# vnminin/phylomap

Measured on NVIDIA B200. Metric: sampled branch-site histories/sec (4-state, 10k-tip tree), higher is better.
Workload: dtype f32

## Files before the change

phylomap_b200/csrc/pm_device.cuh:

```cuda
#pragma once
#include <cstdint>
#include <cuda_runtime.h>

#define PM_NMAX 32
#define PM_DIC_NMAX 8
#define PM_LOCAL_PATH_MAX 64
#define PM_SMEM_POW 8

#define PM_DE_SAMPLE_NA 1u
#define PM_DE_SAMPLE_NEG 2u
#define PM_DE_SAMPLE_ZERO 4u
#define PM_DE_PATH_CAP 8u
#define PM_DE_M_OVERFLOW 16u
#define PM_DE_REPLAY 32u
#define PM_DE_INCONSISTENT 64u
#define PM_DE_BAD_STATE 128u
#define PM_DE_JUMP_LIMIT 256u

namespace pm {

template <typename Real, bool EXACT> struct Ar;
template <> struct Ar<double, true> {
  static __device__ __forceinline__ double mul(double a, double b) { return __dmul_rn(a, b); }
  static __device__ __forceinline__ double add(double a, double b) { return __dadd_rn(a, b); }
// ... 107 lines not shown
    return ((float)(x >> 8) + 0.5f) * (1.0f / 16777216.0f);
  }
};

template <typename Real, bool EXACT> struct StreamSel { typedef StreamD type; };
template <> struct StreamSel<float, false> { typedef StreamF type; };

__device__ __forceinline__ double exp_rand_R(StreamD& g) {
  const double q[16] = {0.6931471805599453, 0.9333736875190459, 0.9888777961838675, 0.9984589039328340,
                        0.9998292811061389, 0.9999833164100727, 0.9999985691438767, 0.9999998906925558,
                        0.9999999924734159, 0.9999999995283275, 0.9999999999728814, 0.9999999999985598,
                        0.9999999999999289, 0.9999999999999968, 0.9999999999999999, 1.0000000000000000};
  double a = 0.;
  double u = g.next();
  while (u <= 0. || u >= 1.) u = g.next();
  for (;;) {
    u = __dadd_rn(u, u);
    if (u > 1.) break;
    a = __dadd_rn(a, q[0]);
  }
  u = __dsub_rn(u, 1.);
  if (u <= q[0]) return __dadd_rn(a, u);
  int i = 0;
  double ustar = g.next(), umin = ustar;
  do {
    ustar = g.next();
    if (umin > ustar) umin = ustar;
    i++;
  } while (u > q[i]);
  return __dadd_rn(a, __dmul_rn(umin, q[0]));
}

template <typename Real, bool EXACT> struct ExpDev;
template <> struct ExpDev<double, true> {
  static __device__ __forceinline__ double draw(StreamD& g) { return exp_rand_R(g); }
};
template <> struct ExpDev<double, false> {
  static __device__ __forceinline__ double draw(StreamD& g) { return -log(g.next()); }
};
template <> struct ExpDev<float, false> {
  static __device__ __forceinline__ float draw(StreamF& g) { return -logf(g.next()); }
};

#define PM_LAMBDA_INV 16

template <typename Real> struct Pin;
template <> struct Pin<float> {
  static __device__ __forceinline__ float mul(float a, float b) { return __fmul_rn(a, b); }
  static __device__ __forceinline__ float add(float a, float b) { return __fadd_rn(a, b); }
  static __device__ __forceinline__ float sub(float a, float b) { return __fsub_rn(a, b); }
  static __device__ __forceinline__ float div(float a, float b) { return __fdiv_rn(a, b); }
  static __device__ __forceinline__ float u01(uint32_t w) { return __fmaf_rn((float)(w >> 9), 1.0f / 8388608.0f, 1.0f / 16777216.0f); }
  static __device__ __forceinline__ float expm(float x) {
    float r;
    asm("ex2.approx.ftz.f32 %0, %1;" : "=f"(r) : "f"(__fmul_rn(x, -1.4426950216293334961f)));
    return r;
  }
  static __device__ __forceinline__ float root(float u, int k) {
    float l, r;
    asm("lg2.approx.ftz.f32 %0, %1;" : "=f"(l) : "f"(u));
    asm("ex2.approx.ftz.f32 %0, %1;" : "=f"(r) : "f"(__fdiv_rn(l, (float)k)));
    return r;
  }
  static __device__ __forceinline__ float neglog(float u) { return -logf(u); }
  static __device__ __forceinline__ int above3(float u, float a, float b, float c) {
    unsigned x, y, z;
    asm("set.gt.u32.f32 %0, %1, %2;" : "=r"(x) : "f"(u), "f"(a));
    asm("set.gt.u32.f32 %0, %1, %2;" : "=r"(y) : "f"(u), "f"(b));
    asm("set.gt.u32.f32 %0, %1, %2;" : "=r"(z) : "f"(u), "f"(c));
    return -(int)(x + y + z);
  }
};
template <> struct Pin<double> {
  static __device__ __forceinline__ double mul(double a, double b) { return __dmul_rn(a, b); }
  static __device__ __forceinline__ double add(double a, double b) { return __dadd_rn(a, b); }
  static __device__ __forceinline__ double sub(double a, double b) { return __dsub_rn(a, b); }
  static __device__ __forceinline__ double div(double a, double b) { return __ddiv_rn(a, b); }
  static __device__ __forceinline__ double u01(uint32_t w) { return ((double)w + 0.5) * (1.0 / 4294967296.0); }
  static __device__ __forceinline__ double expm(double x) { return exp(-x); }
  static __device__ __forceinline__ double root(double u, int k) { return exp2(__ddiv_rn(log2(u), (double)k)); }
  static __device__ __forceinline__ double neglog(double u) { return -log(u); }
  static __device__ __forceinline__ int above3(double u, double a, double b, double c) { return (u > a ? 1 : 0) + (u > b ? 1 : 0) + (u > c ? 1 : 0); }
};

__constant__ float pm_recip[65] = {
    0.f, 1.f, 1.f / 2, 1.f / 3, 1.f / 4, 1.f / 5, 1.f / 6, 1.f / 7, 1.f / 8, 1.f / 9, 1.f / 10, 1.f / 11, 1.f / 12, 1.f / 13,
    1.f / 14, 1.f / 15, 1.f / 16, 1.f / 17, 1.f / 18, 1.f / 19, 1.f / 20, 1.f / 21, 1.f / 22, 1.f / 23, 1.f / 24, 1.f / 25,
    1.f / 26, 1.f / 27, 1.f / 28, 1.f / 29, 1.f / 30, 1.f / 31, 1.f / 32, 1.f / 33, 1.f / 34, 1.f / 35, 1.f / 36, 1.f / 37,
    1.f / 38, 1.f / 39, 1.f / 40, 1.f / 41, 1.f / 42, 1.f / 43, 1.f / 44, 1.f / 45, 1.f / 46, 1.f / 47, 1.f / 48, 1.f / 49,
    1.f / 50, 1.f / 51, 1.f / 52, 1.f / 53, 1.f / 54, 1.f / 55, 1.f / 56, 1.f / 57, 1.f / 58, 1.f / 59, 1.f / 60, 1.f / 61,
    1.f / 62, 1.f / 63, 1.f / 64};

template <typename Real>
__device__ __forceinline__ int poisson_inv(Real lam, uint32_t word) {
  typedef Pin<Real> PN;
  const Real u = PN::u01(word);
  const Real p0 = PN::expm(lam);
  const Real p1 = PN::mul(p0, lam);
  const Real p2 = PN::mul(PN::mul(p1, lam), (Real)0.5);
  const Real c1 = PN::add(p0, p1), c2 = PN::add(c1, p2);
  int k = Pin<Real>::above3(u, p0, c1, c2);
  if (k == 3) {
    Real p = p2, c = c2;
    k = 2;
    while (u > c && k < 64) {
      k++;
      p = PN::mul(PN::mul(p, lam), (Real)pm_recip[k]);
      c = PN::add(c, p);
      if (p < (Real)1e-12 && (Real)k > lam) break;
    }
  }
  return k;
}

template <typename Real>
__device__ __forceinline__ Real next_order_stat(Real x, Real L, int remaining, uint32_t word) {
  const Real u = Pin<Real>::u01(word);
  const Real frac = Pin<Real>::sub((Real)1, remaining == 1 ? u : Pin<Real>::root(u, remaining));
  return Pin<Real>::add(x, Pin<Real>::mul(Pin<Real>::sub(L, x), frac));
}

template <typename Real>
__device__ __forceinline__ Real pos_dec(uint32_t q, Real Le) { return Pin<Real>::mul((Real)q, Pin<Real>::mul(Le, (Real)(1.0 / 65536.0))); }
template <typename Real>
__device__ __forceinline__ uint32_t pos_enc(Real p, Real Le) {
  const Real f = Pin<Real>::add(Pin<Real>::mul(p, Pin<Real>::div((Real)65536, Le)), (Real)0.5);
  return (uint32_t)min(max((int)f, 0), 65535);
}
__device__ __forceinline__ uint32_t pos_rand(uint32_t word) { return min(((word >> 15) + 1u) >> 1, 65535u); }
#define PM_SHAPE(nj, s0, s1) ((uint16_t)((uint32_t)(nj) | ((uint32_t)(s0) << 6) | ((uint32_t)(s1) << 11)))

struct WordStream {
  uint32_t k0, k1, site, iter, slot, hi, j;
  uint32_t o0, o1, o2, o3;
  __device__ __forceinline__ void open(const RngDesc& d, uint32_t local_site, uint32_t it, uint32_t kind, uint32_t idx, uint32_t run) {
    k0 = d.k0; k1 = d.k1; site = d.site0 + local_site; iter = it; slot = make_slot(kind, idx); hi = run << 20; j = 0;
  }
  __device__ __forceinline__ uint32_t next() {
    const uint32_t q = j & 3u;
    if (q == 0u) {
      uint32_t o[4];
      philox4x32_10(hi | (j >> 2), slot, iter, site, k0, k1, o);
      o0 = o[0]; o1 = o[1]; o2 = o[2]; o3 = o[3];
    }
    j++;
    return q == 0u ? o0 : q == 1u ? o1 : q == 2u ? o2 : o3;
  }
};

__device__ __forceinline__ void pair_block(const RngDesc& d, uint32_t local_site, uint32_t it, uint32_t e, uint32_t o[4]) {
  philox4x32_10_rk(e >> 1, make_slot(K_BRPAIR, 0u), it, d.site0 + local_site, d.rk, o);
}

template <typename Real, int NC, bool EXACT, typename U>
__device__ __forceinline__ int categorical(const Real* w, int n, U u, unsigned* err) {
  if (EXACT) {
    Real sum = 0; int npos = 0; unsigned bad = 0;
#pragma unroll
    for (int i = 0; i < n; i++) {
      Real v = w[i];
      if (!isfinite(v)) bad |= PM_DE_SAMPLE_NA;
      else if (v < (Real)0) bad |= PM_DE_SAMPLE_NEG;
      if (v > (Real)0) { npos++; sum = Ar<Real, true>::add(sum, v); }
    }
    if (npos == 0) bad |= PM_DE_SAMPLE_ZERO;
    if (bad) { atomicOr(err, bad); return 0; }
    Real p[NC]; int perm[NC];
#pragma unroll
    for (int i = 0; i < n; i++) { p[i] = Ar<Real, true>::div(w[i], sum); perm[i] = i; }
#pragma unroll
    for (int i = 1; i < n; i++) {
#pragma unroll
      for (int j = i; j >= 1; j--) {
        if (p[j] > p[j - 1]) {
          Real tp = p[j]; p[j] = p[j - 1]; p[j - 1] = tp;
          int ti = perm[j]; perm[j] = perm[j - 1]; perm[j - 1] = ti;
        }
      }
    }
    Real c = 0;
    int pick = -1;
    const int last = perm[n - 1];
#pragma unroll
    for (int j = 0; j < n - 1; j++) {
      c = (j == 0) ? p[0] : Ar<Real, true>::add(c, p[j]);
      if (pick < 0 && (double)u <= (double)c) pick = perm[j];
    }
    return pick < 0 ? last : pick;
  } else {
    Real tot = 0;
#pragma unroll
    for (int i = 0; i < n; i++) tot += w[i];
    if (!(tot > (Real)0) || !isfinite(tot)) { atomicOr(err, tot > (Real)0 ? PM_DE_SAMPLE_NA : PM_DE_SAMPLE_ZERO); return 0; }
    Real t = (Real)u * tot, c = 0;
    int pick = -1, lastpos = 0;
#pragma unroll
    for (int i = 0; i < n; i++) {
      c += w[i];
      if (w[i] > (Real)0) lastpos = i;
      if (pick < 0 && t < c && w[i] > (Real)0) pick = i;
    }
    return pick < 0 ? lastpos : pick;
  }
}

template <typename Real, int NC, bool EXACT>
__device__ __forceinline__ void matvec(const Real* __restrict__ M, int n, Real* v) {
  Real y[NC];
#pragma unroll
  for (int i = 0; i < n; i++) {
    Real acc = 0;
#pragma unroll
    for (int j = 0; j < n; j++) acc = Ar<Real, EXACT>::add(acc, Ar<Real, EXACT>::mul(M[i * n + j], v[j]));
    y[i] = acc;
  }
#pragma unroll
  for (int i = 0; i < n; i++) v[i] = y[i];
}
template <typename Real, int NC, bool EXACT>
__device__ __forceinline__ void matvec_t(const Real* __restrict__ M, int n, Real* v) {
  Real y[NC];
#pragma unroll
  for (int j = 0; j < n; j++) {
    Real acc = 0;
#pragma unroll
    for (int i = 0; i < n; i++) acc = Ar<Real, EXACT>::add(acc, Ar<Real, EXACT>::mul(M[i * n + j], v[i]));
    y[j] = acc;
  }
#pragma unroll
  for (int j = 0; j < n; j++) v[j] = y[j];
}

template <typename Real, int NS> struct VecIO {
  static __device__ __forceinline__ void load(const Real* p, int n, Real* v) { for (int i = 0; i < n; i++) v[i] = p[i]; }
  static __device__ __forceinline__ void store(Real* p, int n, const Real* v) { for (int i = 0; i < n; i++) p[i] = v[i]; }
};
template <> struct VecIO<float, 4> {
  static __device__ __forceinline__ void load(const float* p, int, float* v) {
    float4 t = *reinterpret_cast<const float4*>(p); v[0] = t.x; v[1] = t.y; v[2] = t.z; v[3] = t.w; }
  static __device__ __forceinline__ void store(float* p, int, const float* v) {
    *reinterpret_cast<float4*>(p) = make_float4(v[0], v[1], v[2], v[3]); }
};
template <> struct VecIO<float, 2> {
  static __device__ __forceinline__ void load(const float* p, int, float* v) {
    float2 t = *reinterpret_cast<const float2*>(p); v[0] = t.x; v[1] = t.y; }
  static __device__ __forceinline__ void store(float* p, int, const float* v) {
    *reinterpret_cast<float2*>(p) = make_float2(v[0], v[1]); }
};
template <> struct VecIO<double, 4> {
  static __device__ __forceinline__ void load(const double* p, int, double* v) {
    double2 a = reinterpret_cast<const double2*>(p)[0], b = reinterpret_cast<const double2*>(p)[1];
    v[0] = a.x; v[1] = a.y; v[2] = b.x; v[3] = b.y; }
  static __device__ __forceinline__ void store(double* p, int, const double* v) {
    reinterpret_cast<double2*>(p)[0] = make_double2(v[0], v[1]); reinterpret_cast<double2*>(p)[1] = make_double2(v[2], v[3]); }
};
template <> struct VecIO<double, 2> {
  static __device__ __forceinline__ void load(const double* p, int, double* v) {
    double2 a = *reinterpret_cast<const double2*>(p); v[0] = a.x; v[1] = a.y; }
  static __device__ __forceinline__ void store(double* p, int, const double* v) {
    *reinterpret_cast<double2*>(p) = make_double2(v[0], v[1]); }
};

}
```

phylomap_b200/csrc/pm_kernels.cuh:

```cuda
#pragma once
#include <type_traits>
#include "pm_device.cuh"

namespace pm {

template <typename Real>
struct ChainParams {
  int n, T, E;
  const int* cap_off;
  long long S;
  const Real* model;
  const Real* ppow;
  int jcap;
  const int* up_entries; const int* up_off; int n_up_levels;
  int* rec_cursor;
  const int* cl_entries; const int* cl_warp_off; const int* cl_top_entries; const int* cl_top_off; int n_cl_top_levels;
  const int* cd_top; const int* cd_top_off; int n_cd_top_levels; const int* cd_entries; const int* cd_warp_off;
  const long long* cd_tips; int n_cd_tips;
  const int* down_entries; const int* down_off; int n_down_levels;
  const int* e_parent; const int* e_child; const Real* e_len;
  const long long* maps_off; const double* maps_len;
  int root;
  const uint8_t* tipcode; long long TS;
  uint8_t* node_state; uint32_t* meta; Real* PL;
// ... 774 lines not shown
      cp_async4(slot + PLB + lane4, reinterpret_cast<const char*>(mtb_u) + off64(q0.z, q0.w));
      if (lane < 8) cp_async4(slot + hdst, reinterpret_cast<const char*>(e) + hsrc, lane < 4 || more);
    };
#pragma unroll 1
    for (int u = 0; u < DEPTH; u++) {
      if (i0 + u < i1) { issue(ring + u * SLOT, ep, __ldg(ep), i0 + u + DEPTH < i1); ep += 4; }
      cp_async_commit();
    }
    long long vA = 0, vB = 0, pA = -1, pB = -1;
    int psA = 0, psB = 0;
    if (i0 < i1) {
      cp_async_wait<DEPTH - 1>();
      __syncwarp();
      const int4 h = lds_v4(ring + PLB + 128);
      vA = off64(h.x, h.y); pA = off64(h.z, h.w);
      if (pA >= 0) psA = *reinterpret_cast<const uint8_t*>(nsb_u + (unsigned long long)pA);
    }
    unsigned slot = ring;
    unsigned ring_end = ring + DEPTH * SLOT;
    asm volatile("" : "+r"(ring_end));
    int sprev = 0;
    uint32_t o[4] = {0, 0, 0, 0};
    auto step = [&](int idx, long long v_off, long long p_off, int ps_mem, long long& v_off_n, long long& p_off_n, int& ps_mem_n) {
      const unsigned slot_n = (slot + SLOT == ring_end) ? ring : slot + SLOT;
      cp_async_wait<DEPTH - 2>();
      __syncwarp();
      if (idx + 1 < i1) {
        const int4 h = lds_v4(slot_n + PLB + 128);
        v_off_n = off64(h.x, h.y); p_off_n = off64(h.z, h.w);
        if (h.w >= 0) ps_mem_n = *reinterpret_cast<const uint8_t*>(nsb_u + (unsigned long long)p_off_n);
      }
      if ((idx & 3) == 0 || idx == i0) philox4x32_10_rk((uint32_t)idx >> 2, kslot, iter, gsite, P.rng.rk, o);
      const uint32_t word = (idx & 3) == 0 ? o[0] : (idx & 3) == 1 ? o[1] : (idx & 3) == 2 ? o[2] : o[3];
      Real pl[NS];
      lds_vec<Real, NS>(slot + lanePB, pl);
      const int k = lds_u16(slot + PLB + lane4) - 1;
      const int ps = p_off < 0 ? sprev : ps_mem;
      const int sn = draw_node_state<Real, NS>(P, sBs, sPow, npow_s, k, ps, pl, word);
      if (act) *reinterpret_cast<uint8_t*>(nsb_u + (unsigned long long)v_off) = (uint8_t)sn;
      sprev = sn;
      __syncwarp();
      if (idx + DEPTH < i1) {
        const int4 q0 = lds_v4(slot + PLB + 144);
        __syncwarp();
        issue(slot, ep, q0, idx + 2 * DEPTH < i1);
        ep += 4;
      }
      cp_async_commit();
      slot = slot_n;
    };
#pragma unroll 1
    for (int idx = i0; idx < i1; idx += 2) {
      step(idx, vA, pA, psA, vB, pB, psB);
      if (idx + 1 < i1) step(idx + 1, vB, pB, psB, vA, pA, psA);
    }
    cp_async_wait<0>();
  }
  if (P.n_cd_tips > 0) {
    __syncthreads();
    const int ntip = P.n_cd_tips, ngrp = (ntip + 3) >> 2;
    const uint8_t* const tipb = P.tipcode + site;
    const char* const mtb = reinterpret_cast<const char*>(P.meta + site);
    struct TipLoad { int ps, k, cd; };
    auto load = [&](int grp, TipLoad (&L)[4]) {
#pragma unroll
      for (int q = 0; q < 4; q++) {
        const int v = min(4 * grp + q, ntip - 1);
        const longlong2 en = __ldg(reinterpret_cast<const longlong2*>(P.cd_tips) + v);
        L[q].ps = nst[en.x];
        L[q].k = (int)(*reinterpret_cast<const uint32_t*>(mtb + en.y) & 0xffffu) - 1;
        L[q].cd = tipb[(long long)v * P.TS];
      }
    };
    auto draw = [&](int grp, const TipLoad (&L)[4]) {
      uint32_t o[4];
      philox4x32_10_rk(0x40000000u + (uint32_t)grp, kslot, iter, gsite, P.rng.rk, o);
#pragma unroll
      for (int q = 0; q < 4; q++) {
        if (4 * grp + q < ntip) {
          const uint32_t word = q == 0 ? o[0] : q == 1 ? o[1] : q == 2 ? o[2] : o[3];
          const int sn = draw_tip_state<Real, NS>(P, sBs, sPow, npow_s, L[q].k, L[q].ps, L[q].cd, parity, word);
          if (active) nst[(long long)(4 * grp + q) * S] = (uint8_t)sn;
        }
      }
    };
    TipLoad A[4], B[4];
    int grp = warp;
    if (grp < ngrp) load(grp, A);
    while (grp < ngrp) {
      if (grp + nw < ngrp) load(grp + nw, B);
      draw(grp, A);
      grp += nw;
      if (grp >= ngrp) break;
      if (grp + nw < ngrp) load(grp + nw, A);
      draw(grp, B);
      grp += nw;
    }
  }
}

template <typename Real, int NS, int DEPTH, int MINB>
__global__ void __launch_bounds__(256, MINB) k_nodes_clade(ChainParams<Real> P, uint32_t iter) {
  if (P.ctl) iter = P.ctl[0];
  nodes_clade_block<Real, NS, DEPTH>(P, iter, P.tile_base + (long long)blockIdx.x * 32, (long long)blockIdx.x * 32);
}

__device__ __forceinline__ unsigned long long global_ns() { unsigned long long t; asm volatile("mov.u64 %0, %%globaltimer;" : "=l"(t)); return t; }
__device__ __forceinline__ unsigned sm_id() { unsigned v; asm volatile("mov.u32 %0, %%smid;" : "=r"(v)); return v; }

template <typename Real, int NS, int DEPTH, int MINB>
__global__ void __launch_bounds__(256, MINB) k_prune_nodes_clade(ChainParams<Real> P, uint32_t iter, long long b0, int phases, int* slot_busy,
                                                                 int slots_per_sm, unsigned long long* phase_ns) {
  if (P.ctl) iter = P.ctl[0];
  __shared__ unsigned long long s_t[2];
  __shared__ int s_slot;
  if (threadIdx.x == 0) {
    int slot = (int)blockIdx.x;
    if (slot_busy) {
      const int base = (int)sm_id() * slots_per_sm;
      int k = 0;
      while (atomicCAS(slot_busy + base + k, 0, 1) != 0) k = (k + 1 == slots_per_sm) ? 0 : k + 1;
      slot = base + k;
    }
    s_slot = slot;
    if (phase_ns) s_t[0] = global_ns();
  }
  __syncthreads();
  const int slot = s_slot;
  const long long site0 = (b0 + blockIdx.x) * 32, pl0 = (long long)slot * 32;
  prune_clade_block<Real, NS, DEPTH>(P, site0, pl0);
  __syncthreads();
  if (phases & 2) {
    if (phase_ns && threadIdx.x == 0) s_t[1] = global_ns();
    nodes_clade_block<Real, NS, DEPTH>(P, iter, site0, pl0);
    __syncthreads();
    if (phase_ns && threadIdx.x == 0) {
      const unsigned long long t2 = global_ns();
      atomicAdd(phase_ns, s_t[1] - s_t[0]);
      atomicAdd(phase_ns + 1, t2 - s_t[1]);
    }
  }
  if (threadIdx.x == 0 && slot_busy) atomicExch(slot_busy + slot, 0);
}

#define PM_META(m, q) ((uint32_t)(m) | ((uint32_t)(q) << 16))

template <typename Real>
__device__ __forceinline__ bool rate_ok(Real r) { return isfinite(r) && r > (Real)0; }

__device__ __forceinline__ float lds_real(unsigned a, float) { float v; asm volatile("ld.shared.f32 %0, [%1];" : "=f"(v) : "r"(a)); return v; }
__device__ __forceinline__ double lds_real(unsigned a, double) { double v; asm volatile("ld.shared.f64 %0, [%1];" : "=d"(v) : "r"(a)); return v; }
__device__ __forceinline__ unsigned smem_addr(const void* p) { return (unsigned)__cvta_generic_to_shared(p); }

template <typename Real>
struct EasySmem {
  int cnt, rate, unit, topo;
  __host__ __device__ static int up16(int x) { return (x + 15) & ~15; }
  __host__ __device__ explicit EasySmem(int n) {
    cnt = up16(4 * n * (int)sizeof(double));
    rate = up16(cnt + n * n * (int)sizeof(unsigned));
    unit = up16(rate + n * (int)sizeof(Real));
    topo = up16(unit + n * n * (int)sizeof(Real));
  }
  __host__ __device__ size_t bytes(int chunk) const { return (size_t)topo + (size_t)chunk * 16; }
};
__device__ __forceinline__ void lds_v2s32(unsigned a, int& x, int& y) { asm volatile("ld.shared.v2.s32 {%0,%1}, [%2];" : "=r"(x), "=r"(y) : "r"(a)); }
__device__ __forceinline__ void red_shared_inc(unsigned a) { asm volatile("red.shared.add.u32 [%0], 1;" ::"r"(a) : "memory"); }

template <typename Real, int NS>
__global__ void __launch_bounds__(128, (sizeof(Real) == 8 ? 6 : 8)) k_paths_easy(ChainParams<Real> P, uint32_t iter, int chunk) {
  if (P.ctl) iter = P.ctl[0];
  constexpr int NR = NS > 0 ? NS : 1;
  typedef Pin<Real> PN;
  const int n = NS > 0 ? NS : P.n;
  extern __shared__ __align__(16) unsigned char smem_raw[];
  const EasySmem<Real> lay(n);
  double* s_dw = reinterpret_cast<double*>(smem_raw);
  unsigned* s_cnt = reinterpret_cast<unsigned*>(smem_raw + lay.cnt);
  Real* s_rate = reinterpret_cast<Real*>(smem_raw + lay.rate);
  Real* s_unit = reinterpret_cast<Real*>(smem_raw + lay.unit);
  unsigned char* s_topo = smem_raw + lay.topo;
  const int e0 = blockIdx.y * chunk, e1 = min(P.E, e0 + chunk);
  for (int i = threadIdx.x; i < n * n; i += blockDim.x) { s_cnt[i] = 0; s_unit[i] = (i / n == i % n) ? (Real)1 : (Real)0; }
  for (int i = threadIdx.x; i < n; i += blockDim.x) {
    const Real r = P.model[2 * n * n + 4 * n + i];
    s_rate[i] = rate_ok(r) ? r : (Real)0;
  }
  for (int i = threadIdx.x; i < 4 * n; i += blockDim.x) s_dw[i] = 0.0;
  for (int i = threadIdx.x; i < e1 - e0; i += blockDim.x) {
    int* en = reinterpret_cast<int*>(s_topo + 16 * (size_t)i);
    en[0] = P.e_parent[e0 + i]; en[1] = P.e_child[e0 + i];
    *reinterpret_cast<Real*>(en + 2) = P.e_len[e0 + i];
  }
  __syncthreads();
  unsigned a_base = smem_addr(smem_raw);
  asm volatile("" : "+r"(a_base));
  const unsigned a_cnt = a_base + (unsigned)lay.cnt, a_rate = a_base + (unsigned)lay.rate, a_unit = a_base + (unsigned)lay.unit,
                 a_topo = a_base + (unsigned)lay.topo;
  const long long S = P.S;
  const uint32_t Su = (uint32_t)S;
  const long long site_raw = (long long)blockIdx.x * blockDim.x + threadIdx.x;
  const long long site = site_raw < S ? site_raw : S - 1;
  const bool full = P.full_counts != 0;
  const long long wglob = site_raw >> 5;
  uint32_t* __restrict__ const bal_b = P.hard_ballot + (long long)e0 * P.W + wglob;
  const bool bal_writer = (threadIdx.x & 31) == 0 && wglob < (long long)P.W;
  const uint32_t Wu = (uint32_t)P.W;
  uint32_t* __restrict__ const meta_b = P.meta + (long long)e0 * S + site;
  uint16_t* __restrict__ const shape_b = P.shape + (long long)e0 * S + site;
  uint32_t row = 0, rowf = 0, rowb = 0;
  const uint8_t* __restrict__ nstate = P.node_state + site;
  Real Racc[NR]; double Rsum[NR];
#pragma unroll
  for (int j = 0; j < NR; j++) { Racc[j] = 0; Rsum[j] = 0; }
  auto add_dwell = [&](int s, Real L) {
    if (NS > 0) {
      Real u[NR];
      lds_vec<Real, NS>(a_unit + (unsigned)s * (unsigned)(NR * sizeof(Real)), u);
#pragma unroll
      for (int j = 0; j < NR; j++) Racc[j] = fma(u[j], L, Racc[j]);
    } else if (L != (Real)0) atomicAdd(&s_dw[s], (double)L);
  };
  auto flush_dwell = [&]() {
    if (NS > 0) {
#pragma unroll
      for (int j = 0; j < NR; j++) { Rsum[j] += (double)Racc[j]; Racc[j] = 0; }
    }
  };
  const int nb = e1 - e0;
  struct Ahead { uint32_t mt; int ps, cs; };
  Ahead X = {0, 0, 0}, Y = {0, 0, 0};
  auto fetch = [&](int i, Ahead& a) {
    a.mt = meta_b[rowf]; rowf += Su;
    int par, chi;
    lds_v2s32(a_topo + 16u * (unsigned)i, par, chi);
    a.ps = nstate[(uint64_t)(uint32_t)par * Su];
    a.cs = nstate[(uint64_t)(uint32_t)chi * Su];
  };
  uint32_t po[4] = {0, 0, 0, 0};
  auto body = [&](int i, auto odd_c, auto newblk_c, auto tail_c, const Ahead cur) {
    constexpr bool ODD = decltype(odd_c)::value, NEWBLK = decltype(newblk_c)::value, TAIL = decltype(tail_c)::value;
    const int e = e0 + i;
    const uint32_t mt = cur.mt; const int ps = cur.ps, cs = cur.cs;
    if (NEWBLK) pair_block(P.rng, (uint32_t)site, iter, (uint32_t)e, po);
    const uint32_t wA = ODD ? po[2] : po[0], wB = ODD ? po[3] : po[1];
    const int m = (int)(mt & 0xffffu);
    const uint32_t q = mt >> 16;
    const Real Le = lds_real(a_topo + 16u * (unsigned)i + 8u, (Real)0);
    const bool two = (m == 2) && (ps != cs);
    const Real p1 = pos_dec<Real>(q, Le);
    const Real L0 = two ? p1 : Le;
    const int s0 = two ? ps : cs;
    const Real L1 = two ? PN::sub(Le, p1) : (Real)0;
    const Real lam = PN::add(PN::mul(lds_real(a_rate + (unsigned)sizeof(Real) * (unsigned)s0, (Real)0), L0),
                             PN::mul(lds_real(a_rate + (unsigned)sizeof(Real) * (unsigned)cs, (Real)0), L1));
    const bool hard = (m > 2) || lam > (Real)PM_LAMBDA_INV;
    const bool ok = TAIL ? (!hard && site_raw < S) : !hard;
    const int k = poisson_inv<Real>(lam, wA);
    if (ok && m == 2 && (full || two)) red_shared_inc(a_cnt + 4u * (unsigned)(ps * n + cs));
    add_dwell(s0, ok ? L0 : (Real)0);
    add_dwell(cs, ok ? L1 : (Real)0);
    const uint32_t newq = (!two && k == 1) ? pos_rand(wB) : q;
    if (ok) { meta_b[row] = PM_META((two ? 2 : 1) + k, newq); shape_b[row] = PM_SHAPE(two ? 1 : 0, s0, cs); }
    row += Su;
    const unsigned bal = __ballot_sync(0xffffffffu, TAIL ? (hard && site_raw < S) : hard);
    if (bal_writer) bal_b[rowb] = bal;
    rowb += Wu;
  };
  auto run = [&](auto tail_c) {
    const std::true_type T{}; const std::false_type F{};
    int i = 0;
    if (nb > 0 && (e0 & 1)) {
      fetch(0, X);
      body(0, T, T, tail_c, X);
      i = 1;
    }
    if (i < nb) fetch(i, X);
    if (i + 1 < nb) fetch(i + 1, Y);
    while (i + 3 < nb) {
      const int stop = min(nb - 4, i + 62);
      for (; i <= stop; i += 2) {
        const Ahead cx = X, cy = Y;
        fetch(i + 2, X); fetch(i + 3, Y);
        body(i, F, T, tail_c, cx);
        body(i + 1, T, F, tail_c, cy);
      }
      flush_dwell();
    }
    for (; i + 1 < nb; i += 2) {
      const Ahead cx = X, cy = Y;
      if (i + 2 < nb) fetch(i + 2, X);
      if (i + 3 < nb) fetch(i + 3, Y);
      body(i, F, T, tail_c, cx);
      body(i + 1, T, F, tail_c, cy);
    }
    if (i < nb) body(i, F, T, tail_c, X);
    flush_dwell();
  };
  if ((long long)(blockIdx.x + 1) * blockDim.x <= S) run(std::false_type()); else run(std::true_type());
  if (NS > 0) {
    const int lane = threadIdx.x & 31, warp = threadIdx.x >> 5;
#pragma unroll
    for (int j = 0; j < NR; j++) {
      double v = Rsum[j];
#pragma unroll
      for (int o = 16; o > 0; o >>= 1) v += __shfl_down_sync(0xffffffffu, v, o);
      if (lane == 0) s_dw[warp * n + j] = v;
    }
  }
  __syncthreads();
  const long long blk = (long long)blockIdx.y * gridDim.x + blockIdx.x;
  if ((int)threadIdx.x < n) {
    double v;
    if (NS > 0) { v = 0; for (int w = 0; w < (int)(blockDim.x >> 5); w++) v += s_dw[w * n + threadIdx.x]; }
    else v = s_dw[threadIdx.x];
    P.dw_partial[blk * n + threadIdx.x] = v;
  }
  for (int i = threadIdx.x; i < n * n; i += blockDim.x) if (s_cnt[i]) atomicAdd(&P.cnt[i], (unsigned long long)s_cnt[i]);
}

template <typename Real>
__device__ __forceinline__ Real rate_or_zero(Real r) { return rate_ok(r) ? r : (Real)0; }

template <typename Real>
struct RunPieces {
  Real L, x, rate;
  int left;
  bool gaps;
  bool firstB;
  uint32_t wB;
  WordStream ws;
  bool joint, pend, run0;
  Real v, sc;
  __device__ __forceinline__ void begin(const RngDesc& d, uint32_t site, uint32_t it, uint32_t e, int run, Real len, Real r,
                                       uint32_t cnt_word, bool single_run, uint32_t wordB) {
    L = len; x = 0; rate = r; left = 0; gaps = false; firstB = single_run; wB = wordB; joint = false;
    if (!rate_ok(r)) return;
    const Real lam = Pin<Real>::mul(r, len);
    if (lam > (Real)PM_LAMBDA_INV) { gaps = true; ws.open(d, site, it, K_BRGAP, e, (uint32_t)run); }
    else { left = poisson_inv<Real>(lam, cnt_word); ws.open(d, site, it, K_BRPOS, e, (uint32_t)run); }
  }
  __device__ __forceinline__ void begin_joint(const RngDesc& d, uint32_t site, uint32_t it, uint32_t e, Real len0, int K, Real lam0,
                                             Real lamT, Real r0, uint32_t wordB) {
    typedef Pin<Real> PN;
    L = len0; x = 0; left = K; gaps = false; firstB = true; wB = wordB; joint = true; pend = false; run0 = true;
    v = 0; rate = PN::div(lam0, lamT); sc = PN::div(lamT, r0);
    ws.open(d, site, it, K_BRPOS, e, 0u);
  }
  __device__ __forceinline__ void second_run(Real len1, Real lamT, Real r1) { L = len1; x = 0; run0 = false; sc = Pin<Real>::div(lamT, r1); }
  __device__ __forceinline__ Real next(bool& last) {
    typedef Pin<Real> PN;
    if (joint) {
      if (!pend && left > 0) {
        uint32_t w;
        if (firstB) { w = wB; firstB = false; } else w = ws.next();
        v = next_order_stat<Real>(v, (Real)1, left, w);
        left--; pend = true;
      }
      if (pend && (!run0 || v < rate)) {
        const Real t2 = min(PN::mul(run0 ? v : PN::sub(v, rate), sc), L);
        const Real piece = max(PN::sub(t2, x), (Real)0);
        x = max(t2, x); pend = false; last = false;
        return piece;
      }
      last = true;
      return PN::sub(L, x);
    }
    if (gaps) {
      const Real g = PN::div(PN::neglog(PN::u01(ws.next())), rate);
      const Real t2 = PN::add(x, g);
      if (t2 < L) { x = t2; last = false; return g; }
      last = true;
      return PN::sub(L, x);
    }
    if (left > 0) {
      uint32_t w;
      if (firstB) { w = wB; firstB = false; } else w = ws.next();
      const Real t2 = next_order_stat<Real>(x, L, left, w);
      const Real piece = PN::sub(t2, x);
      x = t2; left--; last = false;
      return piece;
    }
    last = true;
    return PN::sub(L, x);
  }
};

template <typename Real>
__device__ __noinline__ int count_gaps(RngDesc d, uint32_t site, uint32_t it, uint32_t e, uint32_t run, Real L, Real rate, Real* first) {
  typedef Pin<Real> PN;
  WordStream g; g.open(d, site, it, K_BRGAP, e, run);
  Real x = 0; int k = 0;
  for (;;) {
    const Real gp = PN::div(PN::neglog(PN::u01(g.next())), rate);
    const Real t2 = PN::add(x, gp);
    if (!(t2 < L) || k > 70000) break;
    x = t2; k++;
    if (k == 1) *first = gp;
  }
  return k;
}

template <typename Real>
struct HardItem { uint32_t site, e, meta, ends, shape; };

template <typename Real, int NS>
struct PathWorker {
  static constexpr int NC = NS > 0 ? NS : PM_NMAX;
  static constexpr int NR = NS > 0 ? NS : 1;
  typedef typename StreamSel<Real, false>::type Stream;
  typedef Pin<Real> PN;
  const ChainParams<Real>& P;
  const uint32_t iter; const int first; const int n; const bool full;
  const Real* const sB; const Real* const sBs; const Real* const sPow; const int npow_s;
  unsigned* const s_cnt; double* const s_dw;
  const Real* const s_rate_old; const Real* const s_rate_new;
  const Real* __restrict__ rd_len; const uint8_t* __restrict__ rd_st;
  Real* __restrict__ wr_len; uint8_t* __restrict__ wr_st;
  double Rsum[NR];
  unsigned errbits;
  __device__ __forceinline__ PathWorker(const ChainParams<Real>& P_, uint32_t iter_, int first_, int n_, const Real* sB_, const Real* sBs_,
                                        const Real* sPow_, int npow_s_, unsigned* s_cnt_, double* s_dw_, const Real* rate_old_,
                                        const Real* rate_new_)
      : P(P_), iter(iter_), first(first_), n(n_), full(P_.full_counts != 0), sB(sB_), sBs(sBs_), sPow(sPow_), npow_s(npow_s_),
        s_cnt(s_cnt_), s_dw(s_dw_), s_rate_old(rate_old_), s_rate_new(rate_new_), rd_len(P_.rec_len[(iter_ & 1u) ^ 1u]),
        rd_st(P_.rec_st[(iter_ & 1u) ^ 1u]), wr_len(P_.rec_len[iter_ & 1u]), wr_st(P_.rec_st[iter_ & 1u]), errbits(0) {
#pragma unroll
    for (int j = 0; j < NR; j++) Rsum[j] = 0;
  }
  __device__ __forceinline__ void add_dwell(int s, Real L) {
    if (NS > 0) {
#pragma unroll
      for (int j = 0; j < NR; j++) Rsum[j] += (s == j) ? (double)L : 0.0;
    } else atomicAdd(&s_dw[s], (double)L);
  }

  __device__ __forceinline__ void short_item(const HardItem<Real> it, uint32_t& meta_out, uint16_t& shape_out) {
    const long long site = it.site;
    const int eb = (int)it.e;
    const uint32_t mt = it.meta;
    const int m = (int)(mt & 0xffffu);
    const int nj = (int)(it.shape & 0x3fu);
    const int so0 = (int)((it.shape >> 6) & 0x1fu), so1 = (int)((it.shape >> 11) & 0x1fu);
    const int ps = (int)(it.ends & 0xffu), cs = (int)(it.ends >> 8);
    const Real Le = __ldg(P.e_len + eb);
    const uint32_t gsite = P.rng.site0 + (uint32_t)site;
    uint32_t po_old[4], po_new[4];
    pair_block(P.rng, (uint32_t)site, iter, (uint32_t)eb, po_new);
    if (nj < 2) pair_block(P.rng, (uint32_t)site, iter - 1u, (uint32_t)eb, po_old);
    const uint32_t nA = (eb & 1) ? po_new[2] : po_new[0], nB = (eb & 1) ? po_new[3] : po_new[1];
    Real J0, J1, J2;
    if (nj >= 2) {
      const int ck = eb / P.chunk;
      const int cap0 = __ldg(P.cap_off + ck), cap_c = __ldg(P.cap_off + ck + 1) - cap0;
      const long long sl = ((long long)cap0 * P.rec_groups) + (site >> P.rec_shift) * (long long)cap_c;
      const int rd0 = (int)(mt >> 16);
      J0 = rd_len[sl + min(rd0, cap_c - 1)];
// ... 442 lines not shown
```

phylomap_b200/csrc/pm_launch_impl.cuh:

```cuda
#pragma once
#include "pm_launch.cuh"

namespace pm {

template <typename Real, int NS, bool EXACT>
void Sweep<Real, NS, EXACT>::prune(const ChainParams<Real>& P, int grid, size_t smem, cudaStream_t st) {
  if constexpr (!EXACT && (NS == 2 || NS == 4)) {
    constexpr int D = 8, MB = sizeof(Real) == 8 ? 2 : 3;
    const size_t spow = 2 * PM_SMEM_POW * NS * NS * sizeof(Real);
    const size_t sm = spow + (size_t)PM_CLADE_SLOT * 8 * D;
    auto kern = k_prune_clade<Real, NS, D, MB>;
    cudaFuncSetAttribute(kern, cudaFuncAttributeMaxDynamicSharedMemorySize, (int)sm);
    kern<<<grid, 256, sm, st>>>(P);
  }
  else k_prune<Real, NS, EXACT><<<grid, 256, smem, st>>>(P);
}
template <typename Real, int NS, bool EXACT>
void Sweep<Real, NS, EXACT>::nodes(const ChainParams<Real>& P, int grid, size_t smem, cudaStream_t st, uint32_t iter) {
  if constexpr (!EXACT && (NS == 2 || NS == 4)) {
    constexpr int D = 8, MB = sizeof(Real) == 8 ? 2 : 3;
    const size_t sm = smem + (size_t)(32 * NS * sizeof(Real) + 160) * 8 * D;
    auto kern = k_nodes_clade<Real, NS, D, MB>;
    cudaFuncSetAttribute(kern, cudaFuncAttributeMaxDynamicSharedMemorySize, (int)sm);
    kern<<<grid, 256, sm, st>>>(P, iter);
  }
  else k_nodes<Real, NS, EXACT><<<grid, 256, smem, st>>>(P, iter);
}
template <typename Real, int NS, bool EXACT>
struct FusedCfg {
  static constexpr int D = 8, MB = sizeof(Real) == 8 ? 2 : 3;
  static size_t smem(size_t smem_nodes) {
    const size_t sm_prune = 2 * PM_SMEM_POW * (NS > 0 ? NS : 1) * (NS > 0 ? NS : 1) * sizeof(Real) + (size_t)PM_CLADE_SLOT * 8 * D;
    const size_t sm_nodes = smem_nodes + (size_t)(32 * (NS > 0 ? NS : 1) * sizeof(Real) + 160) * 8 * D;
    return sm_prune > sm_nodes ? sm_prune : sm_nodes;
  }
};
template <typename Real, int NS, bool EXACT>
int Sweep<Real, NS, EXACT>::fused_blocks_per_sm(size_t smem_nodes) {
  if constexpr (!EXACT && (NS == 2 || NS == 4)) {
    typedef FusedCfg<Real, NS, EXACT> C;
    auto kern = k_prune_nodes_clade<Real, NS, C::D, C::MB>;
    const size_t sm = C::smem(smem_nodes);
    cudaFuncSetAttribute(kern, cudaFuncAttributeMaxDynamicSharedMemorySize, (int)sm);
    int nb = 0;
    if (cudaOccupancyMaxActiveBlocksPerMultiprocessor(&nb, kern, 256, sm) != cudaSuccess) return 0;
    return nb;
  }
  return 0;
}
template <typename Real, int NS, bool EXACT>
void Sweep<Real, NS, EXACT>::prune_nodes(const ChainParams<Real>& P, int grid, size_t smem_nodes, cudaStream_t st, uint32_t iter,
                                         long long b0, int phases, int* slot_busy, int slots_per_sm, unsigned long long* phase_ns) {
  if constexpr (!EXACT && (NS == 2 || NS == 4)) {
    typedef FusedCfg<Real, NS, EXACT> C;
    auto kern = k_prune_nodes_clade<Real, NS, C::D, C::MB>;
    const size_t sm = C::smem(smem_nodes);
    cudaFuncSetAttribute(kern, cudaFuncAttributeMaxDynamicSharedMemorySize, (int)sm);
    kern<<<grid, 256, sm, st>>>(P, iter, b0, phases, slot_busy, slots_per_sm, phase_ns);
  }
}
template <typename Real, int NS, bool EXACT>
void Sweep<Real, NS, EXACT>::paths(const ChainParams<Real>& P, dim3 grid, size_t smem, cudaStream_t st, uint32_t iter,
                                   int first, int chunk, int hard_blocks) {
  if constexpr (EXACT) k_paths<Real, NS, true><<<grid, 128, smem, st>>>(P, iter, first, chunk);
  else {
    const size_t smem_easy = EasySmem<Real>(P.n).bytes(chunk);
    k_paths_easy<Real, NS><<<grid, 128, smem_easy, st>>>(P, iter, chunk);
    if (!first) k_paths_hard<Real, NS, 8, 0><<<2 * hard_blocks, 128, smem, st>>>(P, iter, first);
    k_paths_hard<Real, NS, 4, 1><<<hard_blocks, 128, smem, st>>>(P, iter, first);
  }
}
template <typename Real, int NS, bool EXACT>
size_t Sweep<Real, NS, EXACT>::small_smem(int T) {
  if constexpr (!EXACT && (NS == 2 || NS == 4)) return (size_t)SmallSmem<Real, NS>(T).total;
  return (size_t)1 << 40;
}
template <typename Real, int NS, bool EXACT>
void Sweep<Real, NS, EXACT>::small_chain(const ChainParams<Real>& P, int sites, cudaStream_t st, uint32_t iter0, int nsweeps,
                                         const SmallOut& out, bool two_per_sm) {
  if constexpr (!EXACT && (NS == 2 || NS == 4)) {
    const size_t sm = (size_t)SmallSmem<Real, NS>(P.T).total;
    auto kern = two_per_sm ? k_small_chain<Real, NS, 2> : k_small_chain<Real, NS, 1>;
    cudaFuncSetAttribute(kern, cudaFuncAttributeMaxDynamicSharedMemorySize, (int)sm);
    kern<<<sites, 256, sm, st>>>(P, iter0, nsweeps, out);
  }
}

}
```

Before: 68.59 billion.

## Cut register pressure in easy path kernel via smem dwell accumulators and hoisted Philox keys

Moves the per-thread dwell accumulators (Racc/Rsum) out of registers into per-thread shared-memory slots, updated with predicated load-add-store. It also replaces the one-hot unit-vector lookup and precomputes the iteration-dependent Philox rounds once per thread (PairBlocks), so each new pair block needs fewer multiplies. Topology is split into an int2 array plus a separate length array, and branches become predicated PTX loads and stores. The aim is lower register use and less divergence and RNG cost, at the price of more shared-memory traffic and a larger smem footprint per block.

```diff
diff --git a/phylomap_b200/csrc/pm_device.cuh b/phylomap_b200/csrc/pm_device.cuh
--- a/phylomap_b200/csrc/pm_device.cuh
+++ b/phylomap_b200/csrc/pm_device.cuh
@@ -283,6 +283,36 @@
   philox4x32_10_rk(e >> 1, make_slot(K_BRPAIR, 0u), it, d.site0 + local_site, d.rk, o);
 }
 
+struct PairBlocks {
+  uint32_t a, k2, k3, k5;
+  static __device__ __forceinline__ void mulw(uint32_t m, uint32_t c, uint32_t& hi, uint32_t& lo) {
+    const uint64_t p = (uint64_t)m * c;
+    hi = (uint32_t)(p >> 32); lo = (uint32_t)p;
+  }
+  __device__ __forceinline__ PairBlocks(const RngDesc& d, uint32_t it) {
+    a = __umulhi(0xCD9E8D57u, it) ^ make_slot(K_BRPAIR, 0u) ^ d.rk[0];
+    k2 = (0xCD9E8D57u * it) ^ d.rk[2];
+    k3 = __umulhi(0xD2511F53u, a) ^ d.rk[3];
+    k5 = (0xD2511F53u * a) ^ d.rk[5];
+  }
+  __device__ __forceinline__ void block(const RngDesc& d, uint32_t j, uint32_t gsite, uint32_t o[4]) const {
+    uint32_t h0, l0, h1, l1;
+    mulw(0xD2511F53u, j, h0, l0);
+    mulw(0xCD9E8D57u, h0 ^ gsite ^ d.rk[1], h1, l1);
+    uint32_t c0 = h1 ^ k2, c1 = l1, c2 = l0 ^ k3, c3;
+    mulw(0xD2511F53u, c0, h0, l0);
+    mulw(0xCD9E8D57u, c2, h1, l1);
+    c0 = h1 ^ c1 ^ d.rk[4]; c2 = h0 ^ k5; c1 = l1; c3 = l0;
+#pragma unroll
+    for (int r = 3; r < 10; r++) {
+      mulw(0xD2511F53u, c0, h0, l0);
+      mulw(0xCD9E8D57u, c2, h1, l1);
+      c0 = h1 ^ c1 ^ d.rk[2 * r]; c2 = h0 ^ c3 ^ d.rk[2 * r + 1]; c1 = l1; c3 = l0;
+    }
+    o[0] = c0; o[1] = c1; o[2] = c2; o[3] = c3;
+  }
+};
+
 template <typename Real, int NC, bool EXACT, typename U>
 __device__ __forceinline__ int categorical(const Real* w, int n, U u, unsigned* err) {
   if (EXACT) {
diff --git a/phylomap_b200/csrc/pm_kernels.cuh b/phylomap_b200/csrc/pm_kernels.cuh
--- a/phylomap_b200/csrc/pm_kernels.cuh
+++ b/phylomap_b200/csrc/pm_kernels.cuh
@@ -950,20 +950,42 @@
 __device__ __forceinline__ double lds_real(unsigned a, double) { double v; asm volatile("ld.shared.f64 %0, [%1];" : "=d"(v) : "r"(a)); return v; }
 __device__ __forceinline__ unsigned smem_addr(const void* p) { return (unsigned)__cvta_generic_to_shared(p); }
 
-template <typename Real>
+template <typename Real, int NS>
 struct EasySmem {
-  int cnt, rate, unit, topo;
+  int cnt, rate, acc, sum, topo;
   __host__ __device__ static int up16(int x) { return (x + 15) & ~15; }
   __host__ __device__ explicit EasySmem(int n) {
     cnt = up16(4 * n * (int)sizeof(double));
     rate = up16(cnt + n * n * (int)sizeof(unsigned));
-    unit = up16(rate + n * (int)sizeof(Real));
-    topo = up16(unit + n * n * (int)sizeof(Real));
-  }
-  __host__ __device__ size_t bytes(int chunk) const { return (size_t)topo + (size_t)chunk * 16; }
+    acc = up16(rate + n * (int)sizeof(Real));
+    sum = acc + (NS > 0 ? NS * 128 * (int)sizeof(Real) : 0);
+    topo = sum + (NS > 0 ? NS * 128 * (int)sizeof(double) : 0);
+  }
+  __host__ __device__ int len(int chunk) const { return topo + chunk * 8; }
+  __host__ __device__ size_t bytes(int chunk) const { return (size_t)len(chunk) + (size_t)chunk * sizeof(Real); }
 };
 __device__ __forceinline__ void lds_v2s32(unsigned a, int& x, int& y) { asm volatile("ld.shared.v2.s32 {%0,%1}, [%2];" : "=r"(x), "=r"(y) : "r"(a)); }
-__device__ __forceinline__ void red_shared_inc(unsigned a) { asm volatile("red.shared.add.u32 [%0], 1;" ::"r"(a) : "memory"); }
+__device__ __forceinline__ void red_shared_inc_if(bool p, unsigned a) {
+  asm volatile("{\n\t.reg .pred q;\n\tsetp.ne.b32 q, %1, 0;\n\t@q red.shared.add.u32 [%0], 1;\n\t}" ::"r"(a), "r"((unsigned)p) : "memory");
+}
+__device__ __forceinline__ void sts_add_if(bool p, unsigned a, float x) {
+  asm volatile("{\n\t.reg .pred q;\n\t.reg .f32 v;\n\tsetp.ne.b32 q, %2, 0;\n\t@q ld.shared.f32 v, [%0];\n\t@q add.rn.f32 v, v, %1;\n\t"
+               "@q st.shared.f32 [%0], v;\n\t}" ::"r"(a), "f"(x), "r"((unsigned)p));
+}
+__device__ __forceinline__ void sts_add_if(bool p, unsigned a, double x) {
+  asm volatile("{\n\t.reg .pred q;\n\t.reg .f64 v;\n\tsetp.ne.b32 q, %2, 0;\n\t@q ld.shared.f64 v, [%0];\n\t@q add.rn.f64 v, v, %1;\n\t"
+               "@q st.shared.f64 [%0], v;\n\t}" ::"r"(a), "d"(x), "r"((unsigned)p));
+}
+__device__ __forceinline__ void sts_real(unsigned a, float x) { asm volatile("st.shared.f32 [%0], %1;" ::"r"(a), "f"(x)); }
+__device__ __forceinline__ void sts_real(unsigned a, double x) { asm volatile("st.shared.f64 [%0], %1;" ::"r"(a), "d"(x)); }
+__device__ __forceinline__ uint32_t ldg_u32(const uint32_t* a) { uint32_t v; asm volatile("ld.global.u32 %0, [%1];" : "=r"(v) : "l"(a)); return v; }
+__device__ __forceinline__ int ldg_u8(const uint8_t* a) { uint32_t v; asm volatile("ld.global.u8 %0, [%1];" : "=r"(v) : "l"(a)); return (int)v; }
+__device__ __forceinline__ void stg_u32_if(bool p, uint32_t* a, uint32_t x) {
+  asm volatile("{\n\t.reg .pred q;\n\tsetp.ne.b32 q, %2, 0;\n\t@q st.global.u32 [%0], %1;\n\t}" ::"l"(a), "r"(x), "r"((unsigned)p));
+}
+__device__ __forceinline__ void stg_u16_if(bool p, uint16_t* a, uint16_t x) {
+  asm volatile("{\n\t.reg .pred q;\n\tsetp.ne.b32 q, %2, 0;\n\t@q st.global.u16 [%0], %1;\n\t}" ::"l"(a), "h"(x), "r"((unsigned)p));
+}
 
 template <typename Real, int NS>
 __global__ void __launch_bounds__(128, (sizeof(Real) == 8 ? 6 : 8)) k_paths_easy(ChainParams<Real> P, uint32_t iter, int chunk) {
@@ -972,79 +994,83 @@
   typedef Pin<Real> PN;
   const int n = NS > 0 ? NS : P.n;
   extern __shared__ __align__(16) unsigned char smem_raw[];
-  const EasySmem<Real> lay(n);
+  const EasySmem<Real, NS> lay(n);
   double* s_dw = reinterpret_cast<double*>(smem_raw);
   unsigned* s_cnt = reinterpret_cast<unsigned*>(smem_raw + lay.cnt);
   Real* s_rate = reinterpret_cast<Real*>(smem_raw + lay.rate);
-  Real* s_unit = reinterpret_cast<Real*>(smem_raw + lay.unit);
-  unsigned char* s_topo = smem_raw + lay.topo;
+  Real* s_acc = reinterpret_cast<Real*>(smem_raw + lay.acc);
+  double* s_sum = reinterpret_cast<double*>(smem_raw + lay.sum);
+  int2* s_topo = reinterpret_cast<int2*>(smem_raw + lay.topo);
+  Real* s_len = reinterpret_cast<Real*>(smem_raw + lay.len(chunk));
   const int e0 = blockIdx.y * chunk, e1 = min(P.E, e0 + chunk);
-  for (int i = threadIdx.x; i < n * n; i += blockDim.x) { s_cnt[i] = 0; s_unit[i] = (i / n == i % n) ? (Real)1 : (Real)0; }
+  for (int i = threadIdx.x; i < n * n; i += blockDim.x) s_cnt[i] = 0;
   for (int i = threadIdx.x; i < n; i += blockDim.x) {
     const Real r = P.model[2 * n * n + 4 * n + i];
     s_rate[i] = rate_ok(r) ? r : (Real)0;
   }
   for (int i = threadIdx.x; i < 4 * n; i += blockDim.x) s_dw[i] = 0.0;
+  if (NS > 0) for (int j = 0; j < NS; j++) { s_acc[j * 128 + threadIdx.x] = 0; s_sum[j * 128 + threadIdx.x] = 0.0; }
   for (int i = threadIdx.x; i < e1 - e0; i += blockDim.x) {
-    int* en = reinterpret_cast<int*>(s_topo + 16 * (size_t)i);
-    en[0] = P.e_parent[e0 + i]; en[1] = P.e_child[e0 + i];
-    *reinterpret_cast<Real*>(en + 2) = P.e_len[e0 + i];
+    s_topo[i] = make_int2(P.e_parent[e0 + i], P.e_child[e0 + i]);
+    s_len[i] = P.e_len[e0 + i];
   }
   __syncthreads();
   unsigned a_base = smem_addr(smem_raw);
   asm volatile("" : "+r"(a_base));
-  const unsigned a_cnt = a_base + (unsigned)lay.cnt, a_rate = a_base + (unsigned)lay.rate, a_unit = a_base + (unsigned)lay.unit,
-                 a_topo = a_base + (unsigned)lay.topo;
+  const unsigned a_cnt = a_base + (unsigned)lay.cnt, a_rate = a_base + (unsigned)lay.rate, a_topo = a_base + (unsigned)lay.topo,
+                 a_len = a_base + (unsigned)lay.len(chunk);
+  const unsigned a_acc = a_base + (unsigned)lay.acc + (unsigned)sizeof(Real) * threadIdx.x,
+                 a_sum = a_base + (unsigned)lay.sum + (unsigned)sizeof(double) * threadIdx.x;
   const long long S = P.S;
-  const uint32_t Su = (uint32_t)S;
+  uint32_t Su = (uint32_t)S;
   const long long site_raw = (long long)blockIdx.x * blockDim.x + threadIdx.x;
   const long long site = site_raw < S ? site_raw : S - 1;
   const bool full = P.full_counts != 0;
   const long long wglob = site_raw >> 5;
-  uint32_t* __restrict__ const bal_b = P.hard_ballot + (long long)e0 * P.W + wglob;
-  const bool bal_writer = (threadIdx.x & 31) == 0 && wglob < (long long)P.W;
-  const uint32_t Wu = (uint32_t)P.W;
-  uint32_t* __restrict__ const meta_b = P.meta + (long long)e0 * S + site;
-  uint16_t* __restrict__ const shape_b = P.shape + (long long)e0 * S + site;
+  uint32_t* __restrict__ bal_b = P.hard_ballot + (long long)e0 * P.W + wglob;
+  unsigned bal_writer = (threadIdx.x & 31) == 0 && wglob < (long long)P.W;
+  uint32_t Wu = (uint32_t)P.W;
+  uint32_t* __restrict__ meta_b = P.meta + (long long)e0 * S + site;
+  uint16_t* __restrict__ shape_b = P.shape + (long long)e0 * S + site;
   uint32_t row = 0, rowf = 0, rowb = 0;
   const uint8_t* __restrict__ nstate = P.node_state + site;
-  Real Racc[NR]; double Rsum[NR];
-#pragma unroll
-  for (int j = 0; j < NR; j++) { Racc[j] = 0; Rsum[j] = 0; }
-  auto add_dwell = [&](int s, Real L) {
-    if (NS > 0) {
-      Real u[NR];
-      lds_vec<Real, NS>(a_unit + (unsigned)s * (unsigned)(NR * sizeof(Real)), u);
-#pragma unroll
-      for (int j = 0; j < NR; j++) Racc[j] = fma(u[j], L, Racc[j]);
-    } else if (L != (Real)0) atomicAdd(&s_dw[s], (double)L);
+  if (sizeof(Real) == 4) asm volatile("" : "+l"(bal_b), "+l"(meta_b), "+l"(shape_b), "+l"(nstate), "+r"(Wu), "+r"(Su), "+r"(bal_writer));
+  auto add_dwell = [&](int s, Real L, bool p) {
+    if (NS > 0) sts_add_if(p, a_acc + (unsigned)s * (unsigned)(128 * sizeof(Real)), L);
+    else if (p && L != (Real)0) atomicAdd(&s_dw[s], (double)L);
   };
   auto flush_dwell = [&]() {
     if (NS > 0) {
 #pragma unroll
-      for (int j = 0; j < NR; j++) { Rsum[j] += (double)Racc[j]; Racc[j] = 0; }
+      for (int j = 0; j < NR; j++) {
+        const unsigned a = a_acc + (unsigned)j * (unsigned)(128 * sizeof(Real)), b = a_sum + (unsigned)j * (128u * 8u);
+        sts_real(b, lds_real(b, 0.0) + (double)lds_real(a, (Real)0));
+        sts_real(a, (Real)0);
+      }
     }
   };
   const int nb = e1 - e0;
   struct Ahead { uint32_t mt; int ps, cs; };
   Ahead X = {0, 0, 0}, Y = {0, 0, 0};
   auto fetch = [&](int i, Ahead& a) {
-    a.mt = meta_b[rowf]; rowf += Su;
+    a.mt = ldg_u32(meta_b + rowf); rowf += Su;
     int par, chi;
-    lds_v2s32(a_topo + 16u * (unsigned)i, par, chi);
-    a.ps = nstate[(uint64_t)(uint32_t)par * Su];
-    a.cs = nstate[(uint64_t)(uint32_t)chi * Su];
+    lds_v2s32(a_topo + 8u * (unsigned)i, par, chi);
+    a.ps = ldg_u8(nstate + (uint64_t)(uint32_t)par * Su);
+    a.cs = ldg_u8(nstate + (uint64_t)(uint32_t)chi * Su);
   };
   uint32_t po[4] = {0, 0, 0, 0};
+  const PairBlocks pb(P.rng, iter);
+  const uint32_t gsite = P.rng.site0 + (uint32_t)site;
   auto body = [&](int i, auto odd_c, auto newblk_c, auto tail_c, const Ahead cur) {
     constexpr bool ODD = decltype(odd_c)::value, NEWBLK = decltype(newblk_c)::value, TAIL = decltype(tail_c)::value;
     const int e = e0 + i;
     const uint32_t mt = cur.mt; const int ps = cur.ps, cs = cur.cs;
-    if (NEWBLK) pair_block(P.rng, (uint32_t)site, iter, (uint32_t)e, po);
+    if (NEWBLK) pb.block(P.rng, (uint32_t)e >> 1, gsite, po);
     const uint32_t wA = ODD ? po[2] : po[0], wB = ODD ? po[3] : po[1];
     const int m = (int)(mt & 0xffffu);
     const uint32_t q = mt >> 16;
-    const Real Le = lds_real(a_topo + 16u * (unsigned)i + 8u, (Real)0);
+    const Real Le = lds_real(a_len + (unsigned)sizeof(Real) * (unsigned)i, (Real)0);
     const bool two = (m == 2) && (ps != cs);
     const Real p1 = pos_dec<Real>(q, Le);
     const Real L0 = two ? p1 : Le;
@@ -1055,14 +1081,15 @@
     const bool hard = (m > 2) || lam > (Real)PM_LAMBDA_INV;
     const bool ok = TAIL ? (!hard && site_raw < S) : !hard;
     const int k = poisson_inv<Real>(lam, wA);
-    if (ok && m == 2 && (full || two)) red_shared_inc(a_cnt + 4u * (unsigned)(ps * n + cs));
-    add_dwell(s0, ok ? L0 : (Real)0);
-    add_dwell(cs, ok ? L1 : (Real)0);
+    red_shared_inc_if(ok && m == 2 && (full || two), a_cnt + 4u * (unsigned)(ps * n + cs));
+    add_dwell(s0, L0, ok);
+    add_dwell(cs, L1, ok && two);
     const uint32_t newq = (!two && k == 1) ? pos_rand(wB) : q;
-    if (ok) { meta_b[row] = PM_META((two ? 2 : 1) + k, newq); shape_b[row] = PM_SHAPE(two ? 1 : 0, s0, cs); }
+    stg_u32_if(ok, meta_b + row, (newq << 16) + (uint32_t)((two ? 2 : 1) + k));
+    stg_u16_if(ok, shape_b + row, (uint16_t)(((uint32_t)cs << 11) + ((uint32_t)s0 << 6) + (two ? 1u : 0u)));
     row += Su;
     const unsigned bal = __ballot_sync(0xffffffffu, TAIL ? (hard && site_raw < S) : hard);
-    if (bal_writer) bal_b[rowb] = bal;
+    stg_u32_if(bal_writer != 0, bal_b + rowb, bal);
     rowb += Wu;
   };
   auto run = [&](auto tail_c) {
@@ -1100,7 +1127,7 @@
     const int lane = threadIdx.x & 31, warp = threadIdx.x >> 5;
 #pragma unroll
     for (int j = 0; j < NR; j++) {
-      double v = Rsum[j];
+      double v = lds_real(a_sum + (unsigned)j * (128u * 8u), 0.0);
 #pragma unroll
       for (int o = 16; o > 0; o >>= 1) v += __shfl_down_sync(0xffffffffu, v, o);
       if (lane == 0) s_dw[warp * n + j] = v;
diff --git a/phylomap_b200/csrc/pm_launch_impl.cuh b/phylomap_b200/csrc/pm_launch_impl.cuh
--- a/phylomap_b200/csrc/pm_launch_impl.cuh
+++ b/phylomap_b200/csrc/pm_launch_impl.cuh
@@ -64,7 +64,7 @@
                                    int first, int chunk, int hard_blocks) {
   if constexpr (EXACT) k_paths<Real, NS, true><<<grid, 128, smem, st>>>(P, iter, first, chunk);
   else {
-    const size_t smem_easy = EasySmem<Real>(P.n).bytes(chunk);
+    const size_t smem_easy = EasySmem<Real, NS>(P.n).bytes(chunk);
     k_paths_easy<Real, NS><<<grid, 128, smem_easy, st>>>(P, iter, chunk);
     if (!first) k_paths_hard<Real, NS, 8, 0><<<2 * hard_blocks, 128, smem, st>>>(P, iter, first);
     k_paths_hard<Real, NS, 4, 1><<<hard_blocks, 128, smem, st>>>(P, iter, first);
```

After: 71.80 billion, median of 6. 1.05x the previous value.
